# KristianHolme/DRiL.jl

Hardware: AMD Instinct MI355X
Metric: env-steps/s (rollout+PPO update) at n_envs=65536 (higher is better)
Workload: dtype f32 (f16x2 split, f32 accumulate)

## Files before the change

dril.jl_amd/csrc/dril_grad_pair.hip:

```cpp
#include <utility>

#include "dril_grad_common.h"
#include "dril_split_pieces.h"

namespace dril {

template <int D, int O> struct PairLds {
    static constexpr int H = 64, DP = FirstLayer<D>::DP, OP = (O + 3) / 4 * 4;
    static constexpr bool WIDE_IN = D > 4;
    static constexpr int W1T = 0, B1 = W1T + DP * H, B2 = B1 + H, W3S = B2 + H, W3B = W3S + O * H, B3 = W3B + O * H, SMALL_END = (B3 + OP + 127) / 128 * 128;
    static constexpr int WIMG = SMALL_END;
    static constexpr int PAIR0 = WIMG + 2 * 2048;
    static constexpr int P1 = 0, P2 = P1 + 2 * 1024, P3 = P2 + 2 * 1024, XI = P3 + (WIDE_IN ? 2 * 1024 : 0), PO = XI + (WIDE_IN ? 2 * 512 : 0);
    static constexpr int RQ = RecLayout<D>::RS == 3 ? 4 : 2, RECB = RQ * 32 * 4;
    static constexpr int REC = (PO + 2 * O * 32 + 3) / 4 * 4, VO = REC + 2 * RECB, VAL = VO + 2 * 64, PAIR_SIZE = (VAL + 2 * 64 + 127) / 128 * 128;
    static constexpr int END = PAIR0 + 2 * PAIR_SIZE;
    static_assert((4 * WIMG) % 512 == 0 && (4 * PAIR0) % 512 == 0 && (4 * PAIR_SIZE) % 512 == 0 && (4 * P2) % 512 == 0, "image bases must be multiples of 512 bytes");
};
__device__ __forceinline__ f16x8 load_frag_W_T(const char* wimg, int tmk, int tmk16, int piece, int mi, int s) {
    const int off = (32 * mi + 16 * s) * 128 + piece * 8192;
    return __builtin_bit_cast(f16x8, frag8(lds_read_tr16(wimg, tmk + off), lds_read_tr16(wimg, tmk16 + off + 4 * 128)));
}

template <int KIND, int O, int HEAD>
__device__ __forceinline__ void grad_body_pair(const GradArgs& a, float* smem) {
    constexpr int D = EnvSpec<KIND>::D, H = 64, MT = 2;
    constexpr bool REC = true, kKeepH1 = HEAD == HEAD_VALUE;
    constexpr float kInvTanhScale = 1.0f / kTanhScale;
    using L = PairLds<D, O>;
#ifdef DRIL_STAMPS_EDGES
    unsigned long long e_[6];
#endif
#ifdef DRIL_STAMPS_EDGES
    { unsigned long long t_; asm volatile("s_memtime %0\n\ts_waitcnt lgkmcnt(0)" : "=s"(t_) :: "memory"); e_[0] = t_; }
#endif
    const int tid = threadIdx.x, lane = tid & 63;
    const int wave = __builtin_amdgcn_readfirstlane(tid >> 6);
    const int w = wave & 1, pr = wave >> 1;
    const int c = lane & 31, h = lane >> 5;
    const NetOff off = HEAD == HEAD_VALUE ? a.critic : a.actor;
    float* wl = smem;
    char* Wimg = reinterpret_cast<char*>(smem + L::WIMG);
    float* pb = smem + L::PAIR0 + pr * L::PAIR_SIZE;
    char* P1 = reinterpret_cast<char*>(pb + L::P1); char* P2 = reinterpret_cast<char*>(pb + L::P2); float* PO = pb + L::PO;
    constexpr int kNT = 256;
    {
        const float* __restrict__ P = a.params;
        for (int i = tid; i < L::DP * H; i += kNT) { const int o = i % H, k = i / H; wl[L::W1T + k * H + o] = k < D ? kTanhScale * P[off.w1 + o + k * H] : 0.0f; }
        for (int i = tid; i < H; i += kNT) { wl[L::B1 + i] = kTanhScale * P[off.b1 + i]; wl[L::B2 + i] = (kTanhScale * kWScale * kActScale) * P[off.b2 + i]; }
        for (int i = tid; i < O * H; i += kNT) { const int o = i % O, k = i / O; const float w3 = P[off.w3 + i]; wl[L::W3S + o * H + k] = w3 * (1.0f / kActScale); wl[L::W3B + o * H + k] = w3 * (1.0f / (kActScale * kActScale)); }
        for (int i = tid; i < L::OP; i += kNT) wl[L::B3 + i] = i < O ? P[off.b3 + i] : 0.0f;
#pragma unroll
        for (int i = tid; i < H * H / 2; i += kNT) {
            const int o = i % H, kp = i / H;
            unsigned hi, lo;
            split2_pair((kTanhScale * kWScale) * P[off.w2 + o + H * (2 * kp)], (kTanhScale * kWScale) * P[off.w2 + o + H * (2 * kp + 1)], hi, lo);
            const int byte = o * 128 + ((((kp >> 2) ^ wimg_g<64>(o)) & 7) << 4) + ((kp & 3) << 2);
            *reinterpret_cast<unsigned*>(Wimg + byte) = hi; *reinterpret_cast<unsigned*>(Wimg + 8192 + byte) = lo;
        }
    }
    if (L::WIDE_IN) { for (int i = tid; i < 2 * L::PAIR_SIZE; i += kNT) { const int q = i % L::PAIR_SIZE; if (q >= L::XI && q < L::PO) smem[L::PAIR0 + i] = 0.f; } }
    __syncthreads();
#ifdef DRIL_STAMPS_EDGES
    { unsigned long long t_; asm volatile("s_memtime %0\n\ts_waitcnt lgkmcnt(0)" : "=s"(t_) :: "memory"); e_[1] = t_; }
#endif

    float adv_mean = 0.f, adv_den = 1.f;
    if (HEAD != HEAD_VALUE && a.normalize_adv) {
        const double s = a.adv_stats[0], q = a.adv_stats[1], n = a.adv_stats[2];
        const double mean = s / n;
        double var = (q - s * mean) / (n - 1.0);
        if (var < 0) var = 0;
        adv_mean = (float)mean; adv_den = (float)sqrt(var) + 1.0e-8f;
    }
    adv_mean = __builtin_bit_cast(float, __builtin_amdgcn_readfirstlane(__builtin_bit_cast(int, adv_mean)));
    const float adv_inv = __builtin_bit_cast(float, __builtin_amdgcn_readfirstlane(__builtin_bit_cast(int, 1.0f / adv_den)));
    float lsr[kLsMax];
#pragma unroll
    for (int o = 0; o < kLsMax; ++o) lsr[o] = 0.f;
    if (HEAD == HEAD_GAUSSIAN) {
#pragma unroll
        for (int o = 0; o < O; ++o) lsr[o] = __builtin_bit_cast(float, __builtin_amdgcn_readfirstlane(__builtin_bit_cast(int, a.params[a.log_std_off + o])));
    }
    const float* ls = lsr;
    const int tbase = wide_tr_base<64>(lane);
    const float sg = __uint_as_float((((__float_as_uint(1.0f / a.invB) >> 23) & 0xffu) + 3u) << 23);
    const float inv_sg = 1.0f / sg;
    GradArgs as = a; as.invB = a.invB * sg;
    lds_char* lds = (lds_char*)smem;
    constexpr int kWimgB = 4 * L::WIMG, kP1B = 4 * L::P1, kP2B = 4 * L::P2, kP3B = 4 * L::P3;
    constexpr int KS = FirstLayer<D>::KS;
    constexpr bool WIDE_IN = L::WIDE_IN;
    constexpr float kObsScale = 16.0f;
    const int pairB = 4 * (L::PAIR0 + pr * L::PAIR_SIZE);
    const int rowc = c * 128 + ((h ^ wimg_g<64>(c)) << 4);
    const int rowP = pairB + rowc;
    const int rowW = rowc + 4096 * w;
    const int ownT = pairB + c * 128 + 8 * h + (((4 * w) ^ wimg_g<64>(c)) << 4);

    f32x16 dW2[MT], dW3acc[O], db2acc, dW1acc[WIDE_IN ? 1 : D], db1acc;
    float db3p[O], dlsp[O], st[5];
#pragma unroll
    for (int r = 0; r < 16; ++r) { db2acc[r] = 0.f; db1acc[r] = 0.f; }
#pragma unroll
    for (int j = 0; j < MT; ++j)
#pragma unroll
        for (int r = 0; r < 16; ++r) dW2[j][r] = 0.f;
#pragma unroll
    for (int d = 0; d < (WIDE_IN ? 1 : D); ++d)
#pragma unroll
        for (int r = 0; r < 16; ++r) dW1acc[d][r] = 0.f;
#pragma unroll
    for (int o = 0; o < O; ++o) {
        db3p[o] = 0.f; dlsp[o] = 0.f;
#pragma unroll
        for (int r = 0; r < 16; ++r) dW3acc[o][r] = 0.f;
    }
#pragma unroll
    for (int i = 0; i < 5; ++i) st[i] = 0.f;

    const int nb = HEAD == HEAD_VALUE ? (int)blockIdx.x - a.G / 2 : (int)blockIdx.x;
    const int GP = HEAD == HEAD_VALUE ? a.Gc : a.G;
    const int g = 2 * nb + pr;
    const int64_t ntiles = (a.count + kTile - 1) / kTile;
    const int64_t g0 = 2 * nb;
    const int64_t trips = g0 < ntiles ? (ntiles - g0 + GP - 1) / GP : 0;
    int64_t tile = g;
    float* RECp = pb + L::REC; float* VOp = pb + L::VO; int* VALp = reinterpret_cast<int*>(pb + L::VAL);
    TileIdx nidx; nidx.gidx = 0; nidx.g32 = 0; nidx.is32 = false; nidx.inb = false;
    if (w == 0) {
        request_records_lds<KIND, HEAD>(a, tile_index(a, tile, ntiles, c), lane, RECp, VOp, VALp);
        nidx = tile_index(a, tile + GP, ntiles, c);
    }
    __syncthreads();
#ifdef DRIL_STAMPS_EDGES
    { unsigned long long t_; asm volatile("s_memtime %0\n\ts_waitcnt lgkmcnt(0)" : "=s"(t_) :: "memory"); e_[2] = t_; }
#endif
#ifdef DRIL_STAMPS
    unsigned long long stamp_acc[10] = {0, 0, 0, 0, 0, 0, 0, 0, 0, 0}, stamp_prev;
    asm volatile("s_memtime %0\n\ts_waitcnt lgkmcnt(0)" : "=s"(stamp_prev) :: "memory");
#endif
    for (int64_t it = 0; it < trips; ++it, tile += GP) {
        const int buf = (int)(it & 1);
        const float* recb = RECp + buf * L::RECB;
        float xk[KS];
#pragma unroll
        for (int s = 0; s < KS; ++s) xk[s] = recb[((((2 * s) >> 2) * 32 + c) << 2) + ((2 * s) & 3) + h];
        if (WIDE_IN && w == 0) {
            unsigned xh[2][4], xl[2][4];
#pragma unroll
            for (int s = 0; s < KS; ++s) {
                const unsigned u = __float_as_uint(xk[s]);
                const auto r = __builtin_amdgcn_permlane32_swap(u, u, false, false);
                const float a0 = 2 * s < D ? kObsScale * __uint_as_float(r[0]) : (2 * s == D ? kObsScale : 0.f), a1 = 2 * s + 1 < D ? kObsScale * __uint_as_float(r[1]) : (2 * s + 1 == D ? kObsScale : 0.f);
                split2_pair(a0, a1, xh[0][s], xl[0][s]);
            }
#pragma unroll
            for (int s = 0; s < 4; ++s) { const float a0 = 8 + 2 * s == D ? kObsScale : 0.f; split2_pair(a0, 0.f, xh[1][s], xl[1][s]); }
            if (h == 0) {
                const int xa = pairB + 4 * L::XI + c * 64;
#pragma unroll
                for (int ch = 0; ch < 2; ++ch) { pl_write(lds, xa + 16 * ch, u32x4{xh[ch][0], xh[ch][1], xh[ch][2], xh[ch][3]}); pl_write(lds, xa + 2048 + 16 * ch, u32x4{xl[ch][0], xl[ch][1], xl[ch][2], xl[ch][3]}); }
            }
        }
        f32x16 h1k;
        {
            f32x16 h1w;
#pragma unroll
            for (int q = 0; q < 4; ++q) {
                const f32x4 b = *reinterpret_cast<const f32x4*>(wl + L::B1 + 32 * w + 8 * q + 4 * h);
                h1w[4 * q + 0] = b[0]; h1w[4 * q + 1] = b[1]; h1w[4 * q + 2] = b[2]; h1w[4 * q + 3] = b[3];
            }
#pragma unroll
            for (int s = 0; s < KS; ++s) h1w = mfma32(wl[L::W1T + (2 * s + h) * H + 32 * w + c], xk[s], h1w);
            tanh16_scaled<false>(h1w, 1.0f);
            pair_store_pieces2<kP1B>(lds, opaque(ownT), h1w);
            if (kKeepH1) h1k = h1w;
        }
        STAMP(0);
        lds_barrier();
        STAMP(1);
        if (w == 0) {
            request_records_lds<KIND, HEAD>(a, nidx, lane, RECp + (buf ^ 1) * L::RECB, VOp + (buf ^ 1) * 64, VALp + (buf ^ 1) * 64);
            nidx = tile_index(a, tile + 2 * GP, ntiles, c);
        }
        f32x16 h2w;
        {
#pragma unroll
            for (int q = 0; q < 4; ++q) {
                const f32x4 b = *reinterpret_cast<const f32x4*>(wl + L::B2 + 32 * w + 8 * q + 4 * h);
                h2w[4 * q + 0] = b[0]; h2w[4 * q + 1] = b[1]; h2w[4 * q + 2] = b[2]; h2w[4 * q + 3] = b[3];
            }
            const int ra = opaque(rowW), rb = opaque(rowP);
#pragma unroll
            for (int ks = 0; ks < 4; ++ks) {
                const int ak = ra ^ (ks << 5), bk = rb ^ (ks << 5);
                f16x8 A[2], B[2];
#pragma unroll
                for (int p = 0; p < 2; ++p) { A[p] = pl_read<f16x8>(lds, ak + kWimgB + p * 8192); B[p] = pl_read<f16x8>(lds, bk + kP1B + p * 4096); }
                h2w = mfma_split3(A[0], A[1], B[0], B[1], h2w);
            }
            tanh16_scaled<true>(h2w, 1.0f / (kWScale * kActScale));
        }
        STAMP(2);
        float out[O], dz[O];
#pragma unroll
        for (int o = 0; o < O; ++o) {
            float p = 0.f;
#pragma unroll
            for (int q = 0; q < 4; ++q) {
                const f32x4 wv = *reinterpret_cast<const f32x4*>(wl + L::W3S + o * H + 32 * w + 8 * q + 4 * h);
                p = fmaf(wv[0], h2w[4 * q + 0], p); p = fmaf(wv[1], h2w[4 * q + 1], p);
                p = fmaf(wv[2], h2w[4 * q + 2], p); p = fmaf(wv[3], h2w[4 * q + 3], p);
            }
            PO[(w * O + o) * 32 + c] = both_halves_sum(p);
        }
        lds_barrier();
        STAMP(3);
        const f32x4 sc = *reinterpret_cast<const f32x4*>(recb + (((RecLayout<D>::RS - 1) * 32 + c) << 2));
        TileIn<O, KS> cur; cur.act = 0; cur.s0 = 0.f; cur.s1 = 0.f;
        const bool valid = VALp[buf * 64 + c] != 0;
        if (HEAD == HEAD_VALUE) { cur.s0 = sc[3]; cur.s1 = a.has_clip_vf ? VOp[buf * 64 + c] : 0.f; }
        else {
            cur.s0 = sc[1]; cur.s1 = sc[2];
            if (HEAD == HEAD_CATEGORICAL) cur.act = __float_as_int(sc[0]) - a.action_start; else cur.xa[0] = sc[0];
        }
#pragma unroll
        for (int o = 0; o < O; ++o) out[o] = (wl[L::B3 + o] + PO[o * 32 + c]) + PO[(O + o) * 32 + c];
        loss_head<O, HEAD>(as, cur, out, valid, h == 0 && w == 0, ls, adv_mean, adv_inv, dz, st, dlsp);
#pragma unroll
        for (int o = 0; o < O; ++o) {
            if (h == 0 && w == 0) db3p[o] += dz[o];
            fma16(dW3acc[o], dz[o], h2w);
        }
#pragma unroll
        for (int q = 0; q < 4; ++q) {
            float dh[4] = {0.f, 0.f, 0.f, 0.f};
#pragma unroll
            for (int o = 0; o < O; ++o) {
                const f32x4 wv = *reinterpret_cast<const f32x4*>(wl + L::W3B + o * H + 32 * w + 8 * q + 4 * h);
#pragma unroll
                for (int cc = 0; cc < 4; ++cc) dh[cc] = fmaf(wv[cc], dz[o], dh[cc]);
            }
#pragma unroll
            for (int cc = 0; cc < 4; ++cc) { const float hv = h2w[4 * q + cc]; h2w[4 * q + cc] = dh[cc] * fmaf(-hv, hv, kActScale * kActScale); }
        }
        add16(db2acc, h2w);
        pair_store_pieces2<kP2B>(lds, opaque(ownT), h2w);
        STAMP(4);
        lds_barrier();
        STAMP(5);
        f32x16 g1;
        {
#pragma unroll
            for (int r = 0; r < 16; ++r) g1[r] = 0.f;
            const int rb = opaque(rowP), tbw = opaque(tbase) ^ (64 * w), tbw16 = tbw ^ 16;
#pragma unroll
            for (int ks = 0; ks < 4; ++ks) {
                const int bk = rb ^ (ks << 5);
                f16x8 A[2], B[2];
#pragma unroll
                for (int p = 0; p < 2; ++p) { A[p] = load_frag_W_T(Wimg, tbw, tbw16, p, ks >> 1, ks & 1); B[p] = pl_read<f16x8>(lds, bk + kP2B + p * 4096); }
                g1 = mfma_split3(A[0], A[1], B[0], B[1], g1);
            }
            f32x16 h1r;
            if (kKeepH1) h1r = h1k; else pair_load_pieces2<kP1B>(lds, opaque(ownT), h1r);
            constexpr float c0 = kInvTanhScale / kWScale, c1 = c0 / (kActScale * kActScale);
            if constexpr (WIDE_IN) {
#pragma unroll
                for (int r = 0; r < 16; ++r) { const float t2 = h1r[r] * h1r[r]; g1[r] = g1[r] * fmaf(-t2, c1, c0); }
            } else {
#pragma unroll
                for (int r = 0; r < 16; ++r) g1[r] = g1[r] * fmaf(-h1r[r], h1r[r], kActScale * kActScale);
            }
        }
        STAMP(6);
        if constexpr (!WIDE_IN) {
            float x4[4];
            { const f32x4 xq = *reinterpret_cast<const f32x4*>(recb + (c << 2)); x4[0] = xq[0]; x4[1] = xq[1]; x4[2] = xq[2]; x4[3] = xq[3]; }
#pragma unroll
            for (int d = 0; d < D; ++d) fma16(dW1acc[d], x4[d], g1);
            add16(db1acc, g1);
        } else {
            pair_store_pieces2<kP3B>(lds, opaque(ownT), g1);
            const int tbw = opaque(tbase) ^ (64 * w), tbw16 = tbw ^ 16;
            const int kh = lane >> 5, gm = (lane >> 4) & 1, e = lane & 15, xq = e >> 2, xp = e & 3;
            const int tx = (8 * kh + xq) * 64 + ((2 * gm + (xp >> 1)) << 4) + 8 * (xp & 1);
            const char* P3 = reinterpret_cast<const char*>(pb + L::P3); const char* XI = reinterpret_cast<const char*>(pb + L::XI);
#pragma unroll
            for (int s = 0; s < 2; ++s) {
                f16x8 Az[2], Bx[2];
#pragma unroll
                for (int p = 0; p < 2; ++p) { Az[p] = __builtin_bit_cast(f16x8, load_frag_wide_T<64>(P3, tbw, tbw16, p, s)); Bx[p] = __builtin_bit_cast(f16x8, load_frag_wide_T<32>(XI, tx, tx, p, s)); }
                dW1acc[0] = mfma_split3(Az[0], Az[1], Bx[0], Bx[1], dW1acc[0]);
            }
        }
        {
            const int tb = opaque(tbase), tbw = tb ^ (64 * w), tbw16 = tbw ^ 16;
            f16x8 Az[2][2];
#pragma unroll
            for (int s = 0; s < 2; ++s)
#pragma unroll
                for (int p = 0; p < 2; ++p) Az[s][p] = __builtin_bit_cast(f16x8, load_frag_wide_T<64>(P2, tbw, tbw16, p, s));
#pragma unroll
            for (int mj = 0; mj < MT; ++mj) {
                f16x8 Bh[2][2];
                const int tbj = tb ^ (64 * mj), tbj16 = tbj ^ 16;
#pragma unroll
                for (int s = 0; s < 2; ++s)
#pragma unroll
                    for (int p = 0; p < 2; ++p) Bh[s][p] = __builtin_bit_cast(f16x8, load_frag_wide_T<64>(P1, tbj, tbj16, p, s));
#pragma unroll
                for (int s = 0; s < 2; ++s) dW2[mj] = mfma_split3(Az[s][0], Az[s][1], Bh[s][0], Bh[s][1], dW2[mj]);
            }
        }
        STAMP(7);
        __syncthreads();
        STAMP(8);
    }
#ifdef DRIL_STAMPS_EDGES
    { unsigned long long t_; asm volatile("s_memtime %0\n\ts_waitcnt lgkmcnt(0)" : "=s"(t_) :: "memory"); e_[3] = t_; }
#endif
#if defined(DRIL_STAMPS) && !defined(DRIL_STAMPS_EDGES)
    if (lane == 0 && a.dbg) {
        unsigned long long* o_ = a.dbg + ((size_t)blockIdx.x * 4 + wave) * 12;
        for (int k = 0; k < 10; ++k) o_[k] = stamp_acc[k];
        o_[10] = (unsigned long long)trips; o_[11] = HEAD;
    }
#endif

    const int SL = HEAD == HEAD_VALUE ? a.slab_c : a.slab_a;
    const int o_w1 = 0, o_b1 = H * D, o_w2 = o_b1 + H, o_b2 = o_w2 + H * H, o_w3 = o_b2 + H, o_b3 = o_w3 + O * H;
    const int o_ls = o_b3 + O, o_st = SL - 8;
    float* slab = (HEAD == HEAD_VALUE ? a.slabs_critic : a.slabs_actor) + (size_t)nb * SL;
    const float inv_s1 = inv_sg * ((kInvTanhScale / kWScale) / (kActScale * kActScale));
    const float inv_sa = inv_sg * (1.0f / kActScale);
    auto emit = [&](auto&& put) {
#pragma unroll
        for (int mj = 0; mj < MT; ++mj)
#pragma unroll
            for (int r = 0; r < 16; ++r) put(o_w2 + 32 * w + rowfn(r, h) + (32 * mj + c) * H, dW2[mj][r] * inv_sa);
        {
            const int rl = lane & 15, unit = 32 * w + rowfn(rl, h);
            const bool wr = (lane & 16) == 0;
            { const float b2 = half_reduce16_lane(db2acc, lane) * inv_sg; if (wr) put(o_b2 + unit, b2); }
            if constexpr (!WIDE_IN) {
                { const float b1 = half_reduce16_lane(db1acc, lane) * inv_s1; if (wr) put(o_b1 + unit, b1); }
#pragma unroll
                for (int d = 0; d < D; ++d) { const float v = half_reduce16_lane(dW1acc[d], lane) * inv_s1; if (wr) put(o_w1 + unit + d * H, v); }
            } else {
#pragma unroll
                for (int r = 0; r < 16; ++r) {
                    const int u_ = 32 * w + rowfn(r, h);
                    const float v = dW1acc[0][r] * (inv_sg * (1.0f / 16.0f));
                    if (c < D) put(o_w1 + u_ + c * H, v); else if (c == D) put(o_b1 + u_, v);
                }
            }
#pragma unroll
            for (int o = 0; o < O; ++o) { const float v = half_reduce16_lane(dW3acc[o], lane) * inv_sa; if (wr) put(o_w3 + o + unit * O, v); }
            static_assert(2 * O + 5 <= 16, "scalar sums: one f32x16");
            f32x16 sc16;
#pragma unroll
            for (int r = 0; r < 16; ++r) sc16[r] = 0.f;
#pragma unroll
            for (int o = 0; o < O; ++o) { sc16[o] = db3p[o]; sc16[O + o] = dlsp[o]; }
#pragma unroll
            for (int k = 0; k < 5; ++k) sc16[2 * O + k] = st[k];
            const float tot = half_reduce16_lane(sc16, lane);
            if (w == 0 && lane < 16) {
                if (lane < O) put(o_b3 + lane, tot * inv_sg);
                else if (lane < 2 * O) { if (HEAD == HEAD_GAUSSIAN) put(o_ls + lane - O, tot * inv_sg); }
                else if (lane < 2 * O + 5) put(o_st + lane - 2 * O, tot);
            }
        }
    };
    const int SLr = (SL + 3) & ~3;
    float* park = smem + pr * SLr;
    __syncthreads();
    emit([&](int i, float v) { park[i] = v; });
    __syncthreads();
#ifdef DRIL_STAMPS_EDGES
    { unsigned long long t_; asm volatile("s_memtime %0\n\ts_waitcnt lgkmcnt(0)" : "=s"(t_) :: "memory"); e_[4] = t_; }
#endif
    const int pad0 = HEAD == HEAD_GAUSSIAN ? o_ls + O : o_ls;
#pragma unroll 6
    for (int i = tid; i < SL; i += 256) {
        const bool pad = (i >= pad0 && i < o_st) || i >= o_st + 5;
        slab[i] = pad ? 0.f : smem[i] + smem[SLr + i];
    }
#ifdef DRIL_STAMPS_EDGES
    { unsigned long long t_; asm volatile("s_memtime %0\n\ts_waitcnt lgkmcnt(0)" : "=s"(t_) :: "memory"); e_[5] = t_; }
#endif
#ifdef DRIL_STAMPS_EDGES
    if (lane == 0 && a.dbg) {
        unsigned long long* o_ = a.dbg + ((size_t)blockIdx.x * 4 + wave) * 12;
        for (int k = 0; k < 5; ++k) o_[k] = e_[k + 1] - e_[k];
        for (int k = 5; k < 10; ++k) o_[k] = 0;
        o_[10] = 1; o_[11] = HEAD;
    }
#endif
}

template <int KIND>
__global__ __launch_bounds__(256, 2) void ppo_grad_pair_kernel(GradArgs a) {
    extern __shared__ __attribute__((aligned(1024))) float smem[];
    if (*a.stop_flag) return;
    constexpr int A = EnvSpec<KIND>::A;
    const bool actor = blockIdx.x < (unsigned)(a.G / 2);
    if (actor) grad_body_pair<KIND, A, EnvSpec<KIND>::discrete ? HEAD_CATEGORICAL : HEAD_GAUSSIAN>(a, smem);
    else grad_body_pair<KIND, 1, HEAD_VALUE>(a, smem);
}

template <int KIND> static size_t grad_pair_lds_bytes() {
    constexpr int D = EnvSpec<KIND>::D, A = EnvSpec<KIND>::A;
    constexpr int wa = PairLds<D, A>::END, wc = PairLds<D, 1>::END;
    return sizeof(float) * (wa > wc ? wa : wc);
}

hipError_t launch_ppo_grad_pair(int kind, const GradArgs& a, hipStream_t s) {
#define CALLP(K) { const size_t lds = grad_pair_lds_bytes<K>(); \
        if (2 * ((a.slab_a + 3) & ~3) > PairLds<EnvSpec<K>::D, EnvSpec<K>::A>::END || 2 * ((a.slab_c + 3) & ~3) > PairLds<EnvSpec<K>::D, 1>::END) return hipErrorInvalidValue;    \
        { hipError_t e = set_max_dynamic_lds((const void*)ppo_grad_pair_kernel<K>, lds); if (e != hipSuccess) return e; } \
        ppo_grad_pair_kernel<K><<<(a.G + a.Gc) / 2, 256, lds, s>>>(a); }
    return with_env_kind<KindShare::Shape>(kind, [&](auto K) -> hipError_t {
        constexpr int KIND = decltype(K)::value;
        CALLP(KIND)
        return hipGetLastError();
    });
#undef CALLP
}

}
```

dril.jl_amd/csrc/dril_split_pieces.h:

```cpp
#pragma once
#include "dril_internal.h"

namespace dril {

template <int H> __device__ __forceinline__ int wimg_g(int n) { return H >= 128 ? (((n & 3) << 2) | ((n >> 2) & 3)) : ((((n >> 1) & 1) << 2) | ((n >> 2) & 3)); }

typedef __attribute__((address_space(3))) char lds_char;
template <class T> __device__ __forceinline__ T pl_read(const lds_char* lds, int byte) { return *reinterpret_cast<const __attribute__((address_space(3))) T*>(lds + byte); }
template <class T> __device__ __forceinline__ void pl_write(lds_char* lds, int byte, T v) { *reinterpret_cast<__attribute__((address_space(3))) T*>(lds + byte) = v; }
template <int IMG> __device__ __forceinline__ void pair_store_pieces2(lds_char* lds, int t, const f32x16& x) {
#pragma unroll
    for (int g = 0; g < 4; ++g) {
        unsigned hi[2], lo[2];
        split2_pair(x[4 * g], x[4 * g + 1], hi[0], lo[0]); split2_pair(x[4 * g + 2], x[4 * g + 3], hi[1], lo[1]);
        const int a = t ^ (g << 4);
        pl_write(lds, a + IMG, u32x2{hi[0], hi[1]}); pl_write(lds, a + IMG + 4096, u32x2{lo[0], lo[1]});
    }
}
__device__ __forceinline__ void pieces_sum2(unsigned hk, unsigned lk, float& x0, float& x1) {
    asm("v_fma_mix_f32 %0, %1, 1.0, %2 op_sel:[0,0,0] op_sel_hi:[1,0,1]" : "=v"(x0) : "v"(hk), "v"(lk));
    asm("v_fma_mix_f32 %0, %1, 1.0, %2 op_sel:[1,0,1] op_sel_hi:[1,0,1]" : "=v"(x1) : "v"(hk), "v"(lk));
}
template <int IMG> __device__ __forceinline__ void pair_load_pieces2(const lds_char* lds, int t, f32x16& x) {
#pragma unroll
    for (int g = 0; g < 4; ++g) {
        const int a = t ^ (g << 4);
        const u32x2 hi = pl_read<u32x2>(lds, a + IMG), lo = pl_read<u32x2>(lds, a + IMG + 4096);
#pragma unroll
        for (int k = 0; k < 2; ++k) {
            const unsigned hk = k ? hi.y : hi.x, lk = k ? lo.y : lo.x;
            float x0, x1; pieces_sum2(hk, lk, x0, x1);
            x[4 * g + 2 * k] = x0; x[4 * g + 2 * k + 1] = x1;
        }
    }
}
__device__ __forceinline__ float both_halves_sum(float v) {
    const unsigned u = __float_as_uint(v);
    const auto r = __builtin_amdgcn_permlane32_swap(u, u, false, false);
    return __uint_as_float(r[0]) + __uint_as_float(r[1]);
}
template <int H>
__device__ __forceinline__ void store_tile_pieces2(char* pimg, int w, const f32x16& x, int lane) {
    constexpr int RB = 2 * H, PS = 32 * RB;
    const int c = lane & 31, h = lane >> 5, rowb = c * RB + 8 * h, gsw = wimg_g<H>(c);
#pragma unroll
    for (int g = 0; g < 4; ++g) {
        unsigned hi[2], lo[2];
        split2_pair(x[4 * g], x[4 * g + 1], hi[0], lo[0]); split2_pair(x[4 * g + 2], x[4 * g + 3], hi[1], lo[1]);
        const int a = rowb + (((4 * w + g) ^ gsw) << 4);
        *reinterpret_cast<u32x2*>(pimg + a) = u32x2{hi[0], hi[1]}; *reinterpret_cast<u32x2*>(pimg + PS + a) = u32x2{lo[0], lo[1]};
    }
}
template <int H>
__device__ __forceinline__ void load_tile_pieces2(const char* pimg, int w, f32x16& x, int lane) {
    constexpr int RB = 2 * H, PS = 32 * RB;
    const int c = lane & 31, h = lane >> 5, rowb = c * RB + 8 * h, gsw = wimg_g<H>(c);
#pragma unroll
    for (int g = 0; g < 4; ++g) {
        const int a = rowb + (((4 * w + g) ^ gsw) << 4);
        const u32x2 hi = *reinterpret_cast<const u32x2*>(pimg + a), lo = *reinterpret_cast<const u32x2*>(pimg + PS + a);
#pragma unroll
        for (int k = 0; k < 2; ++k) {
            const unsigned hk = k ? hi.y : hi.x, lk = k ? lo.y : lo.x;
            float x0, x1; pieces_sum2(hk, lk, x0, x1);
            x[4 * g + 2 * k] = x0; x[4 * g + 2 * k + 1] = x1;
        }
    }
}
template <int H>
__device__ __forceinline__ int wide_trm_base(int lane) {
    static_assert(H >= 128, "wide_trm_base: the four-bit chunk swizzle of rows >= 256 bytes");
    constexpr int RB = 2 * H;
    const int h = lane >> 5, gm = (lane >> 4) & 1, e = lane & 15, q = e >> 2, p = e & 3, n = 4 * h + q;
    return n * RB + ((((2 * gm + (p >> 1)) ^ wimg_g<H>(n)) & 15) << 4) + 8 * (p & 1);
}
template <int H>
__device__ __forceinline__ void load_tile_pieces2_T(const char* pimg, int tm, f32x16& x) {
    constexpr int RB = 2 * H, PS = 32 * RB;
    static_assert((8 * RB) % 64 == 0 && PS % 64 == 0, "offsets must leave bits 0-5 alone");
    const int tm32 = tm ^ 32;
#pragma unroll
    for (int Q = 0; Q < 4; ++Q) {
        const int a = ((Q & 1) ? tm32 : tm) + 8 * Q * RB;
        const u32x2 hi = __builtin_bit_cast(u32x2, lds_read_tr16(pimg, a)), lo = __builtin_bit_cast(u32x2, lds_read_tr16(pimg, a + PS));
        float x0, x1, x2, x3;
        pieces_sum2(hi.x, lo.x, x0, x1); pieces_sum2(hi.y, lo.y, x2, x3);
        x[4 * Q] = x0; x[4 * Q + 1] = x1; x[4 * Q + 2] = x2; x[4 * Q + 3] = x3;
    }
}
template <int H>
__device__ __forceinline__ int wide_tr_base(int lane) {
    constexpr int RB = 2 * H;
    const int kh = lane >> 5, gm = (lane >> 4) & 1, e = lane & 15, q = e >> 2, p = e & 3, n = 8 * kh + q;
    return n * RB + ((((2 * gm + (p >> 1)) ^ wimg_g<H>(n)) & 15) << 4) + 8 * (p & 1);
}
template <int H>
__device__ __forceinline__ bf16x8 load_frag_wide_T(const char* pimg, int tm, int tm16, int piece, int s) {
    constexpr int RB = 2 * H, PS = 32 * RB;
    const int off = 16 * s * RB + piece * PS;
    static_assert((16 * RB) % 32 == 0 && PS % 32 == 0, "offsets must leave bits 0-4 alone");
    return frag8(lds_read_tr16(pimg, tm + off), lds_read_tr16(pimg, tm16 + off + 4 * RB));
}

}
```

Measured before the change: 410.7 million.

## Permute W2 hidden-unit order so each wave consumes its own h2 pieces in registers

Reorders the k index of the W2 half-precision image with a bit permutation so a wave's own activation tile lines up with an MFMA K-slice. The wave can then feed half of the backward g1 product straight from registers before the barrier, and only the partner's half is read from LDS afterwards. Also changes the piece store layout and moves the B2 bias load earlier. The aim is less LDS traffic and less work waiting behind the barrier. The cost is more complex index permutations, including in the dW2 writeback, with a risk of subtle layout bugs.

```diff
diff --git a/dril.jl_amd/csrc/dril_grad_pair.hip b/dril.jl_amd/csrc/dril_grad_pair.hip
--- a/dril.jl_amd/csrc/dril_grad_pair.hip
+++ b/dril.jl_amd/csrc/dril_grad_pair.hip
@@ -17,9 +17,9 @@
     static constexpr int END = PAIR0 + 2 * PAIR_SIZE;
     static_assert((4 * WIMG) % 512 == 0 && (4 * PAIR0) % 512 == 0 && (4 * PAIR_SIZE) % 512 == 0 && (4 * P2) % 512 == 0, "image bases must be multiples of 512 bytes");
 };
-__device__ __forceinline__ f16x8 load_frag_W_T(const char* wimg, int tmk, int tmk16, int piece, int mi, int s) {
-    const int off = (32 * mi + 16 * s) * 128 + piece * 8192;
-    return __builtin_bit_cast(f16x8, frag8(lds_read_tr16(wimg, tmk + off), lds_read_tr16(wimg, tmk16 + off + 4 * 128)));
+__device__ __forceinline__ f16x8 load_frag_W_T(const char* wimg, int tmk, int tmk32, int piece, int s) {
+    const int off = 16 * s * 128 + piece * 8192;
+    return __builtin_bit_cast(f16x8, frag8(lds_read_tr16(wimg, tmk + off), lds_read_tr16(wimg, tmk32 + off + 8 * 128)));
 }
 
 template <int KIND, int O, int HEAD>
@@ -55,7 +55,8 @@
             const int o = i % H, kp = i / H;
             unsigned hi, lo;
             split2_pair((kTanhScale * kWScale) * P[off.w2 + o + H * (2 * kp)], (kTanhScale * kWScale) * P[off.w2 + o + H * (2 * kp + 1)], hi, lo);
-            const int byte = o * 128 + ((((kp >> 2) ^ wimg_g<64>(o)) & 7) << 4) + ((kp & 3) << 2);
+            const int kq = pair_kperm(2 * kp) >> 1;
+            const int byte = o * 128 + ((((kq >> 2) ^ wimg_g<64>(o)) & 7) << 4) + ((kq & 3) << 2);
             *reinterpret_cast<unsigned*>(Wimg + byte) = hi; *reinterpret_cast<unsigned*>(Wimg + 8192 + byte) = lo;
         }
     }
@@ -83,7 +84,7 @@
         for (int o = 0; o < O; ++o) lsr[o] = __builtin_bit_cast(float, __builtin_amdgcn_readfirstlane(__builtin_bit_cast(int, a.params[a.log_std_off + o])));
     }
     const float* ls = lsr;
-    const int tbase = wide_tr_base<64>(lane);
+    const int tbase = wide_tr_base<64>(lane), tbaseW = pair_trk_base(lane);
     const float sg = __uint_as_float((((__float_as_uint(1.0f / a.invB) >> 23) & 0xffu) + 3u) << 23);
     const float inv_sg = 1.0f / sg;
     GradArgs as = a; as.invB = a.invB * sg;
@@ -164,6 +165,8 @@
             }
         }
         f32x16 h1k;
+        f32x16 h2w;
+        const int rao = opaque(rowW) ^ (w << 6), rbo = opaque(rowP) ^ (w << 6);
         {
             f32x16 h1w;
 #pragma unroll
@@ -174,7 +177,14 @@
 #pragma unroll
             for (int s = 0; s < KS; ++s) h1w = mfma32(wl[L::W1T + (2 * s + h) * H + 32 * w + c], xk[s], h1w);
             tanh16_scaled<false>(h1w, 1.0f);
-            pair_store_pieces2<kP1B>(lds, opaque(ownT), h1w);
+#pragma unroll
+            for (int q = 0; q < 4; ++q) {
+                const f32x4 b = *reinterpret_cast<const f32x4*>(wl + L::B2 + 32 * w + 8 * q + 4 * h);
+                h2w[4 * q + 0] = b[0]; h2w[4 * q + 1] = b[1]; h2w[4 * q + 2] = b[2]; h2w[4 * q + 3] = b[3];
+            }
+            u32x4 ph[2], pl[2];
+            split_pieces_k(h1w, ph, pl);
+            pair_store_pieces_k<kP1B>(lds, rbo, ph, pl);
             if (kKeepH1) h1k = h1w;
         }
         STAMP(0);
@@ -184,17 +194,11 @@
             request_records_lds<KIND, HEAD>(a, nidx, lane, RECp + (buf ^ 1) * L::RECB, VOp + (buf ^ 1) * 64, VALp + (buf ^ 1) * 64);
             nidx = tile_index(a, tile + 2 * GP, ntiles, c);
         }
-        f32x16 h2w;
-        {
-#pragma unroll
-            for (int q = 0; q < 4; ++q) {
-                const f32x4 b = *reinterpret_cast<const f32x4*>(wl + L::B2 + 32 * w + 8 * q + 4 * h);
-                h2w[4 * q + 0] = b[0]; h2w[4 * q + 1] = b[1]; h2w[4 * q + 2] = b[2]; h2w[4 * q + 3] = b[3];
-            }
-            const int ra = opaque(rowW), rb = opaque(rowP);
-#pragma unroll
-            for (int ks = 0; ks < 4; ++ks) {
-                const int ak = ra ^ (ks << 5), bk = rb ^ (ks << 5);
+        {
+#pragma unroll
+            for (int t = 0; t < 4; ++t) {
+                const int s = t & 1, x_ = t >= 2 ? 64 : 0;
+                const int ak = rao ^ x_ ^ (s << 5), bk = rbo ^ x_ ^ (s << 5);
                 f16x8 A[2], B[2];
 #pragma unroll
                 for (int p = 0; p < 2; ++p) { A[p] = pl_read<f16x8>(lds, ak + kWimgB + p * 8192); B[p] = pl_read<f16x8>(lds, bk + kP1B + p * 4096); }
@@ -233,6 +237,7 @@
             if (h == 0 && w == 0) db3p[o] += dz[o];
             fma16(dW3acc[o], dz[o], h2w);
         }
+        const int tbo = opaque(tbaseW) ^ (4160 * w), tbo32 = tbo ^ 32;
 #pragma unroll
         for (int q = 0; q < 4; ++q) {
             float dh[4] = {0.f, 0.f, 0.f, 0.f};
@@ -246,25 +251,35 @@
             for (int cc = 0; cc < 4; ++cc) { const float hv = h2w[4 * q + cc]; h2w[4 * q + cc] = dh[cc] * fmaf(-hv, hv, kActScale * kActScale); }
         }
         add16(db2acc, h2w);
-        pair_store_pieces2<kP2B>(lds, opaque(ownT), h2w);
+        f32x16 g1;
+        {
+#pragma unroll
+            for (int r = 0; r < 16; ++r) g1[r] = 0.f;
+            f16x8 A[2][2];
+#pragma unroll
+            for (int s = 0; s < 2; ++s)
+#pragma unroll
+                for (int p = 0; p < 2; ++p) A[s][p] = load_frag_W_T(Wimg, tbo, tbo32, p, s);
+            u32x4 ph[2], pl[2];
+            split_pieces_k(h2w, ph, pl);
+            pair_store_pieces_k<kP2B>(lds, rbo, ph, pl);
+#pragma unroll
+            for (int s = 0; s < 2; ++s) g1 = mfma_split3(A[s][0], A[s][1], __builtin_bit_cast(f16x8, ph[s]), __builtin_bit_cast(f16x8, pl[s]), g1);
+        }
         STAMP(4);
         lds_barrier();
         STAMP(5);
-        f32x16 g1;
-        {
-#pragma unroll
-            for (int r = 0; r < 16; ++r) g1[r] = 0.f;
-            const int rb = opaque(rowP), tbw = opaque(tbase) ^ (64 * w), tbw16 = tbw ^ 16;
-#pragma unroll
-            for (int ks = 0; ks < 4; ++ks) {
-                const int bk = rb ^ (ks << 5);
+        {
+#pragma unroll
+            for (int s = 0; s < 2; ++s) {
+                const int bk = rbo ^ 64 ^ (s << 5);
                 f16x8 A[2], B[2];
 #pragma unroll
-                for (int p = 0; p < 2; ++p) { A[p] = load_frag_W_T(Wimg, tbw, tbw16, p, ks >> 1, ks & 1); B[p] = pl_read<f16x8>(lds, bk + kP2B + p * 4096); }
+                for (int p = 0; p < 2; ++p) { A[p] = load_frag_W_T(Wimg, tbo ^ 4096, tbo32 ^ 4096, p, s); B[p] = pl_read<f16x8>(lds, bk + kP2B + p * 4096); }
                 g1 = mfma_split3(A[0], A[1], B[0], B[1], g1);
             }
             f32x16 h1r;
-            if (kKeepH1) h1r = h1k; else pair_load_pieces2<kP1B>(lds, opaque(ownT), h1r);
+            if (kKeepH1) h1r = h1k; else pair_load_pieces_k<kP1B>(lds, rbo, h1r);
             constexpr float c0 = kInvTanhScale / kWScale, c1 = c0 / (kActScale * kActScale);
             if constexpr (WIDE_IN) {
 #pragma unroll
@@ -339,7 +354,7 @@
 #pragma unroll
         for (int mj = 0; mj < MT; ++mj)
 #pragma unroll
-            for (int r = 0; r < 16; ++r) put(o_w2 + 32 * w + rowfn(r, h) + (32 * mj + c) * H, dW2[mj][r] * inv_sa);
+            for (int r = 0; r < 16; ++r) put(o_w2 + 32 * w + pair_kperm(rowfn(r, h)) + (32 * mj + pair_kperm(c)) * H, dW2[mj][r] * inv_sa);
         {
             const int rl = lane & 15, unit = 32 * w + rowfn(rl, h);
             const bool wr = (lane & 16) == 0;
diff --git a/dril.jl_amd/csrc/dril_split_pieces.h b/dril.jl_amd/csrc/dril_split_pieces.h
--- a/dril.jl_amd/csrc/dril_split_pieces.h
+++ b/dril.jl_amd/csrc/dril_split_pieces.h
@@ -33,6 +33,38 @@
             x[4 * g + 2 * k] = x0; x[4 * g + 2 * k + 1] = x1;
         }
     }
+}
+__host__ __device__ constexpr int pair_kperm(int u) { return (u & ~12) | ((u & 4) << 1) | ((u & 8) >> 1); }
+__device__ __forceinline__ void split_pieces_k(const f32x16& x, u32x4 (&hi)[2], u32x4 (&lo)[2]) {
+#pragma unroll
+    for (int s = 0; s < 2; ++s) {
+        unsigned hk[4], lk[4];
+#pragma unroll
+        for (int k = 0; k < 4; ++k) split2_pair(x[8 * s + 2 * k], x[8 * s + 2 * k + 1], hk[k], lk[k]);
+        hi[s] = u32x4{hk[0], hk[1], hk[2], hk[3]}; lo[s] = u32x4{lk[0], lk[1], lk[2], lk[3]};
+    }
+}
+template <int IMG> __device__ __forceinline__ void pair_store_pieces_k(lds_char* lds, int t, const u32x4 (&hi)[2], const u32x4 (&lo)[2]) {
+#pragma unroll
+    for (int s = 0; s < 2; ++s) {
+        const int a = t ^ (s << 5);
+        pl_write(lds, a + IMG, u32x2{hi[s].x, hi[s].y}); pl_write(lds, a + IMG + 4096, u32x2{lo[s].x, lo[s].y});
+        pl_write(lds, a + IMG + 8, u32x2{hi[s].z, hi[s].w}); pl_write(lds, a + IMG + 4096 + 8, u32x2{lo[s].z, lo[s].w});
+    }
+}
+template <int IMG> __device__ __forceinline__ void pair_load_pieces_k(const lds_char* lds, int t, f32x16& x) {
+#pragma unroll
+    for (int s = 0; s < 2; ++s) {
+        const int a = t ^ (s << 5);
+        const u32x4 hi = pl_read<u32x4>(lds, a + IMG), lo = pl_read<u32x4>(lds, a + IMG + 4096);
+        const unsigned hk[4] = {hi.x, hi.y, hi.z, hi.w}, lk[4] = {lo.x, lo.y, lo.z, lo.w};
+#pragma unroll
+        for (int k = 0; k < 4; ++k) { float x0, x1; pieces_sum2(hk[k], lk[k], x0, x1); x[8 * s + 2 * k] = x0; x[8 * s + 2 * k + 1] = x1; }
+    }
+}
+__device__ __forceinline__ int pair_trk_base(int lane) {
+    const int kh = lane >> 5, gm = (lane >> 4) & 1, e = lane & 15, q = e >> 2, p = e & 3, n = 4 * kh + q;
+    return n * 128 + ((((2 * gm + (p & 1)) ^ wimg_g<64>(n)) & 7) << 4) + 8 * (p >> 1);
 }
 __device__ __forceinline__ float both_halves_sum(float v) {
     const unsigned u = __float_as_uint(v);
```

Result: no change. 414.6 million, median of 6 (+0.9%).
